# bcc-research/CFMMRouter.jl

Measured on AMD Instinct MI355X. Metric: find_arb! pools/sec + route! wall-clock, 1M-pool arbitrage, 1/2/4/8 GPU, higher is better.
Workload: dtype f64; 1 GPU; config3: 1M mixed ProductTwoCoin + GeometricMeanTwoCoin pools (500k each), 256 tokens, LinearNonnegative arbitrage; pools_per_gpu=1000000, pools_total=1000000, variant=materialising, full=False

## Files before the change

### cfmmrouter.jl_amd/csrc/ops_two_coin.h

```cpp
#pragma once

#include "fast_arith.h"

#include <type_traits>

namespace cfmm {

struct Trade {
    double d1, d2, l1, l2;
};

struct Px {
    double v1, v2, y1, y2, yg, dlv;
};

constexpr int kDirNone = 0, kDir1 = 1, kDir2 = 2, kDirBoth = 3;
__device__ __forceinline__ void expand_dir(int dir, double d, double l, Trade& t)
{
    if (dir == kDirBoth) return;
    t.d1 = dir == kDir1 ? d : 0.0;
    t.d2 = dir == kDir2 ? d : 0.0;
    t.l1 = dir == kDir2 ? l : 0.0;
    t.l2 = dir == kDir1 ? l : 0.0;
}

typedef unsigned int stream_u2 __attribute__((ext_vector_type(2), may_alias));
typedef unsigned int stream_u4 __attribute__((ext_vector_type(4), may_alias));
template <bool LEAN, class T, class I>
__device__ __forceinline__ T stream_at(const T* base, I i)
{
    if constexpr (LEAN) {
        static_assert(sizeof(T) == 8 || sizeof(T) == 16, "pool streams are 8- or 16-byte records");
        using Bits = typename std::conditional<sizeof(T) == 8, stream_u2, stream_u4>::type;
        const Bits bits = *reinterpret_cast<const Bits*>(reinterpret_cast<const char*>(base) + (size_t)((uint32_t)i * (uint32_t)sizeof(T)));
        T out;
        __builtin_memcpy(&out, &bits, sizeof(T));
        return out;
    } else {
        return base[i];
    }
}

template <bool LEAN = false, class I>
__device__ __forceinline__ int2 load_packed(const PackedFeeTok* pk, I i)
{
    const PackedFeeTok k = stream_at<LEAN>(pk, i);
    return make_int2((int)k.tok, (int)k.gidx);
}
__device__ __forceinline__ double load_packed_fee(int gbase, const double* fee) { return gbase < 0 ? *fee : 0.0; }
template <bool FAST, bool LEAN = false>
__device__ __forceinline__ void resolve_packed(int gbase, const double2* gtab_lds, int2& ai, double& g, double& yg)
{
    const unsigned tok = (unsigned)ai.x;
    if (LEAN || gbase >= 0) {
        const double2 gy = gtab_lds[gbase + ai.y];
        g = gy.x;
        yg = pinned(gy.y);
    } else if constexpr (FAST) {
        yg = rcp_refined(g);
    }
    ai = make_int2((int)(tok & 0xffffu), (int)(tok >> 16));
}

struct ProductOps {
    static constexpr bool kNeedsLogPrices = false;
    static constexpr bool kPrefetch = true;
    struct Raw {
        double2 R;
        double g;
        int2 ai;
        double yg;
    };
    ProductPools p;
    template <bool GBINS, bool LEAN = false, class I>
    __device__ __forceinline__ Raw load(I i) const
    {
        Raw r;
        r.R = stream_at<LEAN>(p.R, i);
        r.yg = 0.0;
        if constexpr (GBINS) {
            r.g = p.gamma[i];
            r.ai = p.Ai[i];
        } else {
            r.ai = load_packed<LEAN>(p.pk, i);
            r.g = LEAN ? 0.0 : load_packed_fee(p.gbase, p.gamma + i);
        }
        return r;
    }
    template <bool GBINS, bool FAST, bool LEAN = false>
    __device__ __forceinline__ void resolve(Raw& r, const double2* gtab_lds) const
    {
        if constexpr (!GBINS) resolve_packed<FAST, LEAN>(p.gbase, gtab_lds, r.ai, r.g, r.yg);
    }
    __device__ __forceinline__ int2 tokens(const Raw& r) const { return r.ai; }
    __device__ __forceinline__ void solve_full(double R1, double R2, double g, double v1, double v2, Trade& t) const
    {
        const double k = R1 * R2;
        const double m12 = v2 / v1;
        const double m21 = v1 / v2;
        const double gm12 = g * m12;
        const double gm21 = g * m21;
        t.d1 = max0(sqrt(gm12 * k) - R1) / g;
        t.d2 = max0(sqrt(gm21 * k) - R2) / g;
        t.l1 = max0(R1 - sqrt(k / gm21));
        t.l2 = max0(R2 - sqrt(k / gm12));
    }

    template <bool FAST>
    __device__ __forceinline__ int solve_dir(const Raw& r, const Px& px, double& d, double& l, Trade& t) const
    {
        const double R1 = r.R.x, R2 = r.R.y, g = r.g, v1 = px.v1, v2 = px.v2;
        constexpr double kMargin = 1.0 + 1e-12;
        const double a = v1 * R1, b = v2 * R2;
        const bool p1 = (g * b) * kMargin >= a;
        const bool p2 = (g * a) * kMargin >= b;
        d = l = 0.0;
        if (p1 != p2) {
            const double k = R1 * R2;
            const double r_in = p1 ? R1 : R2, r_out = p1 ? R2 : R1;
            if constexpr (FAST) {
                const double gm = g * div_by(p1 ? v2 : v1, p1 ? v1 : v2, p1 ? px.y1 : px.y2);
                d = div_by(__builtin_fmax(fast_sqrt(gm * k) - r_in, 0.0), g, px.yg);
                l = __builtin_fmax(r_out - fast_sqrt(fast_div(k, gm)), 0.0);
            } else {
                const double gm = g * ((p1 ? v2 : v1) / (p1 ? v1 : v2));
                d = max0(sqrt(gm * k) - r_in) / g;
                l = max0(r_out - sqrt(k / gm));
            }
            return p1 ? kDir1 : kDir2;
        }
        if (p1 || a != a || b != b) {
            solve_full(R1, R2, g, v1, v2, t);
            return kDirBoth;
        }
        return kDirNone;
    }
};

__device__ __forceinline__ double geom_arb_delta(double m, double r1, double r2, double eta, double g)
{
    const double inner = (((g * m) * eta) * r1) * pow(r2, eta);
    return max0(pow(inner, 1.0 / (eta + 1.0)) - r2) / g;
}
__device__ __forceinline__ double geom_arb_lambda(double m, double r1, double r2, double eta, double g)
{
    const double base = (r2 * pow(r1, 1.0 / eta)) / ((eta * g) * m);
    return max0(r1 - pow(base, eta / (1.0 + eta)));
}

struct GeoMeanOps {
    static constexpr bool kNeedsLogPrices = false;
    static constexpr bool kPrefetch = true;
    struct Raw {
        double2 R, w;
        double g;
        int2 ai;
        double yg;
    };
    GeoMeanPools p;
    template <bool GBINS, bool LEAN = false, class I>
    __device__ __forceinline__ Raw load(I i) const { return Raw{p.R[i], p.w[i], p.gamma[i], p.Ai[i], 0.0}; }
    template <bool GBINS, bool FAST, bool LEAN = false>
    __device__ __forceinline__ void resolve(Raw&, const double2*) const {}
    __device__ __forceinline__ int2 tokens(const Raw& r) const { return r.ai; }
    template <bool FAST>
    __device__ __forceinline__ int solve_dir(const Raw& r, const Px& px, double& d, double& l, Trade& t) const
    {
        d = l = 0.0;
        const double v1 = px.v1, v2 = px.v2;
        const double R1 = r.R.x, R2 = r.R.y, g = r.g;
        const double eta = r.w.x / r.w.y;
        const double ieta = 1.0 / eta;
        const double m12 = v2 / v1, m21 = v1 / v2;
        constexpr double kMargin = 1.0 + 1e-11;
        const bool p1 = (((g * m12) * eta) * R2) * kMargin >= R1;
        const bool p2 = (((g * m21) * ieta) * R1) * kMargin >= R2;
        t.d1 = t.d2 = t.l1 = t.l2 = 0.0;
        if (p1 != p2) {
            const double m = p1 ? m12 : m21, e = p1 ? eta : ieta;
            const double ra = p1 ? R2 : R1, rb = p1 ? R1 : R2;
            const double dx = geom_arb_delta(m, ra, rb, e, g);
            const double lx = geom_arb_lambda(m, ra, rb, e, g);
            t.d1 = p1 ? dx : 0.0;
            t.d2 = p1 ? 0.0 : dx;
            t.l1 = p1 ? 0.0 : lx;
            t.l2 = p1 ? lx : 0.0;
        } else if (p1) {
            t.d1 = geom_arb_delta(m12, R2, R1, eta, g);
            t.d2 = geom_arb_delta(m21, R1, R2, ieta, g);
            t.l1 = geom_arb_lambda(m21, R1, R2, ieta, g);
            t.l2 = geom_arb_lambda(m12, R2, R1, eta, g);
        }
        return kDirBoth;
    }
};

struct GeoMeanLogOps {
    static constexpr bool kNeedsLogPrices = true;
    static constexpr bool kPrefetch = true;
    struct Raw {
        double2 R, Q;
        double eta, g;
        int2 ai;
        double yg;
    };
    GeoMeanPools p;
    template <bool GBINS, bool LEAN = false, class I>
    __device__ __forceinline__ Raw load(I i) const
    {
        Raw r;
        r.R = stream_at<LEAN>(p.R, i);
        r.Q = stream_at<LEAN>(p.Q, i);
        r.eta = stream_at<LEAN>(p.eta, i);
        r.yg = 0.0;
        if constexpr (GBINS) {
            r.g = p.gamma[i];
            r.ai = p.Ai[i];
        } else {
            r.ai = load_packed<LEAN>(p.pk, i);
            r.g = LEAN ? 0.0 : load_packed_fee(p.gbase, p.gamma + i);
        }
        return r;
    }
    template <bool GBINS, bool FAST, bool LEAN = false>
    __device__ __forceinline__ void resolve(Raw& r, const double2* gtab_lds) const
    {
        if constexpr (!GBINS) resolve_packed<FAST, LEAN>(p.gbase, gtab_lds, r.ai, r.g, r.yg);
    }
    __device__ __forceinline__ int2 tokens(const Raw& r) const { return r.ai; }
    template <bool FAST>
    __device__ __forceinline__ void one_direction(const Raw& r, const Px& px, bool dir1, double n, double dd, double& d, double& l) const
    {
        const double R1 = r.R.x, R2 = r.R.y, g = r.g, eta = r.eta;
        const double ra = dir1 ? R2 : R1, rb = dir1 ? R1 : R2;
        const double A = dir1 ? (r.Q.x + px.dlv) : (r.Q.y - eta * px.dlv);
        double X, Y;
        if constexpr (FAST) {
            X = fast_exp(fast_div(A, eta + 1.0));
            Y = fast_div((X * ra) * dd, n);
            d = div_by(max0(X - rb), g, px.yg);
        } else {
            X = exp(A / (eta + 1.0));
            Y = ((X * ra) * dd) / n;
            d = max0(X - rb) / g;
        }
        l = max0(ra - Y);
    }
    template <bool FAST>
    __device__ __forceinline__ int solve_dir(const Raw& r, const Px& px, double& d, double& l, Trade& t) const
    {
        const double v1 = px.v1, v2 = px.v2;
        const double R1 = r.R.x, R2 = r.R.y, g = r.g;
        const double eta = r.eta;
        const double n1 = ((g * v2) * eta) * R2, d1 = v1;
        const double n2 = (g * v1) * R1, d2 = v2 * eta;
        const bool p1 = n1 > R1 * d1, p2 = n2 > R2 * d2;
        d = l = 0.0;
        if (v1 != v1 || v2 != v2) { t.d1 = t.d2 = t.l1 = t.l2 = v1 + v2; return kDirBoth; }
        if (!(p1 || p2)) return kDirNone;
        one_direction<FAST>(r, px, p1, p1 ? n1 : n2, p1 ? d1 : d2, d, l);
        if (!(p1 && p2)) return p1 ? kDir1 : kDir2;
        t.d1 = d;
        t.l2 = l;
        one_direction<FAST>(r, px, false, n2, d2, t.d2, t.l1);
        return kDirBoth;
    }
};

struct SolidlyOps : ProductOps {
    template <bool FAST>
    __device__ __forceinline__ int solve_dir(const Raw& r, const Px& px, double& d, double& l, Trade& t) const
    {
        const double R1 = r.R.x, R2 = r.R.y, g = r.g, v1 = px.v1, v2 = px.v2;
        d = l = 0.0;
        if (v1 != v1 || v2 != v2) { t.d1 = t.d2 = t.l1 = t.l2 = v1 + v2; return kDirBoth; }
        const double s1 = R1 * R1, s2 = R2 * R2;
        const double A = v2 * (R2 * __builtin_fma(3.0, s1, s2));
        const double B = v1 * (R1 * __builtin_fma(3.0, s2, s1));
        const bool p1 = g * A > B, p2 = A < g * B;
        if (!(p1 || p2)) return kDirNone;
        const double va = p1 ? v1 : v2, vb = p1 ? v2 : v1;
        const double ra = p1 ? R1 : R2, rb = p1 ? R2 : R1;
        const double num = __builtin_fma(-g, vb, va), den = __builtin_fma(g, vb, va);
        const double c = cbrt(num / den);
        const double c2 = c * c;
        const double tt = (va * ((1.0 + c) + c2)) / ((g * vb) * ((1.0 - c) + c2));
        const double t0 = rb / ra;
        const double rho = (t0 * __builtin_fma(t0, t0, 1.0)) / (tt * __builtin_fma(tt, tt, 1.0));
        const double xa = ra * sqrt(sqrt(rho));
        d = max0(xa - ra) / g;
        l = max0(rb - tt * xa);
        return p1 ? kDir1 : kDir2;
    }
};

}
```

### cfmmrouter.jl_amd/csrc/sweep_core.h

```cpp
#pragma once

#include "granule.h"
#include "ops_two_coin.h"
#include "ops_univ3.h"

#include <type_traits>

namespace cfmm {

typedef double d2v __attribute__((ext_vector_type(2)));
__device__ __forceinline__ void store_pair(double2* dst, double x, double y, int nt)
{
    d2v val = {x, y};
    if (nt) asm volatile("global_store_dwordx4 %0, %1, off nt\n\ts_nop 1" : : "v"(dst), "v"(val) : "memory");
    else asm volatile("global_store_dwordx4 %0, %1, off sc1\n\ts_nop 1" : : "v"(dst), "v"(val) : "memory");
}
__device__ __forceinline__ void store_pair_at(double2* base, uint32_t i, double x, double y)
{
    d2v val = {x, y};
    asm volatile("s_nop 4\n\tglobal_store_dwordx4 %0, %1, %2 sc1\n\ts_nop 1" : : "v"(i * 16u), "v"(val), "s"(base) : "memory");
}

__device__ __forceinline__ void store_row(double* dst, double x)
{
    asm volatile("global_store_dwordx2 %0, %1, off sc1" : : "v"(dst), "v"(x) : "memory");
}

struct SweepLds {
    double2* vy;
    double2* gtab;
    double* lv;
    double* bins;
    double* wsum;
    double* flags;
    double* my_bins;
};

template <int BLOCK, bool GBINS>
__device__ __forceinline__ SweepLds carve_lds(const SweepArgs& a)
{
    extern __shared__ __attribute__((aligned(16))) double lds[];
    SweepLds L;
    if constexpr (GBINS) {
        L.vy = nullptr;
        L.gtab = nullptr;
        L.lv = L.bins = L.my_bins = L.flags = nullptr;
        L.wsum = lds;
        return L;
    }
    L.vy = reinterpret_cast<double2*>(lds);
    L.gtab = reinterpret_cast<double2*>(lds + ((size_t)a.n_pad << (a.v_shift - 3)));
    L.lv = reinterpret_cast<double*>(L.gtab + a.gtab_n);
    L.bins = L.lv + (a.need_logv ? a.n_pad : 0);
    L.wsum = L.bins + (size_t)a.copies * a.n_pad;
    L.flags = L.wsum + BLOCK / 64;
    L.my_bins = L.bins + (size_t)(a.copies == 1 ? 0 : (threadIdx.x >> 6)) * a.n_pad;
    return L;
}

__device__ __forceinline__ int wait_armed(const SweepArgs& a)
{
    const long long t0 = (long long)wall_clock64();
    for (;;) {
        const unsigned long long w = __hip_atomic_load(a.arm_word, __ATOMIC_RELAXED, __HIP_MEMORY_SCOPE_SYSTEM);
        if (w == a.arm_seq) return 1;
        if ((w & ~kArmCancel) > a.arm_seq || w == (a.arm_seq | kArmCancel)) return 0;
        if ((long long)wall_clock64() - t0 > a.arm_timeout) return -1;
        __builtin_amdgcn_s_sleep(1);
    }
}

__device__ __forceinline__ void report(const SweepArgs& a, unsigned long long bit)
{
    if (a.flags && threadIdx.x == 0) __hip_atomic_fetch_or(a.flags, bit, __ATOMIC_RELAXED, __HIP_MEMORY_SCOPE_SYSTEM);
}

constexpr int kStageLive = 1, kStageFast = 2, kStageGaveUp = 4;
constexpr int kPricePre = 2;
struct PricePre {
    double p[kPricePre];
};
template <int BLOCK>
__device__ __forceinline__ PricePre request_prices(const double* v, int n)
{
    PricePre r;
#pragma unroll
    for (int k = 0; k < kPricePre; ++k) {
        const int j = (int)threadIdx.x + k * BLOCK;
        r.p[k] = v[j < n ? j : n - 1];
    }
    return r;
}
template <int BLOCK, bool GBINS, bool PRE = false>
__device__ __forceinline__ int stage_prices(const SweepArgs& a, const SweepLds& L, const PricePre& pre = PricePre{})
{
    if constexpr (GBINS) {
        __syncthreads();
        return kStageLive;
    }
    const int tid = threadIdx.x;
    const int n_zero = a.copies * a.n_pad;
    const bool logs = a.need_logv != 0;
    const bool armed = a.arm_word != nullptr;
    bool live = true, gave_up = false;
    if (armed) {
        for (int j = tid; j < n_zero; j += BLOCK) L.bins[j] = 0.0;
        for (int j = tid; j < a.gtab_n; j += BLOCK) {
            const double g = a.gtab[j];
            L.gtab[j] = make_double2(g, rcp_refined(g));
        }
        if (tid == 0) L.flags[BLOCK / 64] = (double)wait_armed(a);
        __syncthreads();
        live = L.flags[BLOCK / 64] > 0.0;
        gave_up = L.flags[BLOCK / 64] < 0.0;
    }
    bool in_window = true;
    for (int j = tid, k = 0; j < a.n; j += BLOCK, ++k) {
        double vj;
        if (armed) vj = __hip_atomic_load(a.v + j, __ATOMIC_RELAXED, __HIP_MEMORY_SCOPE_SYSTEM);
        else if (PRE && k < kPricePre) vj = k == 0 ? pre.p[0] : pre.p[1];
        else vj = a.v[j];
        if (a.v_shift == 4) L.vy[j] = make_double2(vj, rcp_refined(vj));
        else reinterpret_cast<double*>(L.vy)[j] = vj;
        in_window = in_window && in_fast_window(vj);
        if (logs) L.lv[j] = log(vj);
    }
    if (!armed) {
        for (int j = tid; j < n_zero; j += BLOCK) L.bins[j] = 0.0;
        for (int j = tid; j < a.gtab_n; j += BLOCK) {
            const double g = a.gtab[j];
            L.gtab[j] = make_double2(g, rcp_refined(g));
        }
    }
    const bool wave_in = __all(in_window ? 1 : 0) != 0;
    if ((tid & 63) == 0) L.flags[tid >> 6] = wave_in ? 1.0 : 0.0;
    __syncthreads();
    bool all_in = true;
#pragma unroll
    for (int w = 0; w < BLOCK / 64; ++w) all_in = all_in && L.flags[w] != 0.0;
    return (live ? kStageLive : 0) | (all_in ? kStageFast : 0) | (gave_up ? kStageGaveUp : 0);
}

template <class Ops, bool MAT, bool GBINS, bool FAST, bool LEAN, class Idx>
__device__ __forceinline__ void process_pool(const Ops& ops, const SweepArgs& a, const SweepLds& L,
                                             const typename Ops::Raw& raw_in, Idx i, double& acc)
{
    const auto put_record = [&](double x, double y) {
        if constexpr (LEAN) store_pair_at(a.Delta, i, x, y);
        else store_pair(a.Delta + i, x, y, a.nt_stores);
    };
    typename Ops::Raw raw = raw_in;
    ops.template resolve<GBINS, FAST, LEAN>(raw, L.gtab);
    const int2 tok = ops.tokens(raw);
    Px px;
    px.yg = raw.yg;
    if constexpr (GBINS) {
        px.v1 = a.v[tok.x];
        px.v2 = a.v[tok.y];
        px.y1 = px.y2 = 0.0;
        px.dlv = Ops::kNeedsLogPrices ? log(px.v2 / px.v1) : 0.0;
    } else {
        if constexpr (FAST) {
            const double2 a1 = L.vy[tok.x], a2 = L.vy[tok.y];
            px.v1 = a1.x; px.y1 = a1.y;
            px.v2 = a2.x; px.y2 = a2.y;
        } else {
            const char* base = reinterpret_cast<const char*>(L.vy);
            px.v1 = *reinterpret_cast<const double*>(base + ((size_t)tok.x << a.v_shift));
            px.v2 = *reinterpret_cast<const double*>(base + ((size_t)tok.y << a.v_shift));
            px.y1 = px.y2 = 0.0;
        }
        px.dlv = 0.0;
        if constexpr (Ops::kNeedsLogPrices)
            px.dlv = a.need_logv ? L.lv[tok.y] - L.lv[tok.x] : log(px.v2 / px.v1);
    }
    Trade t;
    double d, l;
    int dir;
    dir = ops.template solve_dir<FAST>(raw, px, d, l, t);
    const double v1 = px.v1, v2 = px.v2;
    const bool one = dir == kDir1 || dir == kDir2;
    const bool plain = one && (!MAT || !a.compact || (__double2hiint(d) | __double2hiint(l)) >= 0);
    if (plain) {
        const bool d1 = dir == kDir1;
        if (MAT) {
            if (a.compact) {
                put_record(d1 ? d : -d, l);
            } else {
                store_pair(a.Delta + i, d1 ? d : 0.0, d1 ? 0.0 : d, a.nt_stores);
                store_pair(a.Lambda + i, d1 ? 0.0 : l, d1 ? l : 0.0, a.nt_stores);
            }
        }
        acc += l * (d1 ? v2 : v1) - d * (d1 ? v1 : v2);
        if constexpr (GBINS) {
            a.gflow[i] = d1 ? make_double2(0.0 - d, l) : make_double2(l, 0.0 - d);
        } else {
            const double f_in = 0.0 - d;
            if (f_in != 0.0) atomicAdd(&L.my_bins[d1 ? tok.x : tok.y], f_in);
            if (l != 0.0) atomicAdd(&L.my_bins[d1 ? tok.y : tok.x], l);
        }
        return;
    }
    if (dir == kDirNone) {
        if (MAT) {
            if (a.compact) {
                put_record(0.0, 0.0);
            } else {
                store_pair(a.Delta + i, 0.0, 0.0, a.nt_stores);
                store_pair(a.Lambda + i, 0.0, 0.0, a.nt_stores);
            }
        }
        if constexpr (GBINS) a.gflow[i] = make_double2(0.0, 0.0);
        return;
    }
    expand_dir(dir, d, l, t);
    if (MAT) {
        if (a.compact) {
            const int d1h = __double2hiint(t.d1), d2h = __double2hiint(t.d2), l1h = __double2hiint(t.l1), l2h = __double2hiint(t.l2);
            const int z1 = d2h | __double2loint(t.d2) | l1h | __double2loint(t.l1);
            const int z2 = d1h | __double2loint(t.d1) | l2h | __double2loint(t.l2);
            const bool dir1 = (z1 == 0) & ((d1h | l2h) >= 0);
            const bool dir2 = (z2 == 0) & ((d2h | l1h) >= 0);
            double ra = t.d1, rb = t.l2;
            if (!dir1) {
                if (dir2) {
                    ra = -t.d2;
                    rb = t.l1;
                } else {
                    a.Lambda[i] = make_double2(t.d1, t.d2);
                    a.Over[i] = make_double2(t.l1, t.l2);
                    ra = 0.0;
                    rb = -1.0;
                }
            }
            put_record(ra, rb);
        } else {
            store_pair(a.Delta + i, t.d1, t.d2, a.nt_stores);
            store_pair(a.Lambda + i, t.l1, t.l2, a.nt_stores);
        }
    }
    acc += (t.l1 * v1 + t.l2 * v2) - (t.d1 * v1 + t.d2 * v2);
    const double f1 = t.l1 - t.d1, f2 = t.l2 - t.d2;
    if constexpr (GBINS) {
        a.gflow[i] = make_double2(f1, f2);
    } else {
        if (f1 != 0.0) atomicAdd(&L.my_bins[tok.x], f1);
        if (f2 != 0.0) atomicAdd(&L.my_bins[tok.y], f2);
    }
}

template <class Ops, bool MAT, int BLOCK, bool GBINS, bool FAST, bool PREFETCH, bool LEAN, class Idx>
__device__ __forceinline__ void tile_loop(const Ops& ops, const SweepArgs& a, const SweepLds& L, typename Ops::Raw cur,
                                          Idx i, Idx step, Idx left, double& acc)
{
    if constexpr (PREFETCH) {
        bool ok = left > 0;
        while (ok) {
            const bool more = left > 1;
            typename Ops::Raw nxt = cur;
            if (more) nxt = ops.template load<GBINS, LEAN>((Idx)(i + step));
            process_pool<Ops, MAT, GBINS, FAST, LEAN>(ops, a, L, cur, i, acc);
            i += step;
            --left;
            ok = more;
            cur = nxt;
        }
    } else {
        bool ok = left > 0;
        while (ok) {
            process_pool<Ops, MAT, GBINS, FAST, LEAN>(ops, a, L, cur, i, acc);
            i += step;
            ok = --left > 0;
            if (ok) cur = ops.template load<GBINS, LEAN>(i);
        }
    }
}

constexpr int kArithFull = 0, kArithFast = 1, kArithAuto = 2;
template <class Ops, bool MAT, int BLOCK, bool GBINS, int FASTK, bool MULTI, bool LEAN, class Idx>
__device__ __forceinline__ double sweep_tiles(const Ops& ops, const SweepArgs& a, const SweepLds& L, const typename Ops::Raw& cur,
                                              Idx i, Idx step, Idx left, bool& poison, bool& live, const PricePre& pre)
{
    static_assert(!(GBINS && FASTK != kArithFull), "large-market mode runs on the compiler's sequences");
    double acc = 0.0;
    const int staged = stage_prices<BLOCK, GBINS, !GBINS>(a, L, pre);
    poison = (staged & kStageLive) == 0;
    live = !poison || (staged & kStageGaveUp) != 0;
    if (staged & kStageGaveUp) report(a, kFlagGaveUp);
    if (FASTK == kArithFast && !poison && (staged & kStageFast) == 0) {
        poison = true;
        report(a, kFlagWindow);
    }
    if (poison) left = 0;
    constexpr bool kPre = Ops::kPrefetch && !MULTI;
    if constexpr (FASTK == kArithAuto) {
        if (staged & kStageFast) tile_loop<Ops, MAT, BLOCK, GBINS, true, kPre, LEAN>(ops, a, L, cur, i, step, left, acc);
        else tile_loop<Ops, MAT, BLOCK, GBINS, false, kPre, LEAN>(ops, a, L, cur, i, step, left, acc);
    } else {
        tile_loop<Ops, MAT, BLOCK, GBINS, FASTK == kArithFast, kPre, LEAN>(ops, a, L, cur, i, step, left, acc);
    }
    return acc;
}

typedef unsigned long long u2v __attribute__((ext_vector_type(2)));
__device__ __forceinline__ void publish_column(const SweepArgs& a, int j, double val)
{
    if (a.direct_host.gran) {
        u2v g = {granule(a.direct_host.tag, val, 0), granule(a.direct_host.tag, val, 1)};
        asm volatile("global_store_dwordx4 %0, %1, off sc0 sc1\n\ts_nop 1" : : "v"(a.direct_host.gran + 2 * (size_t)j), "v"(g) : "memory");
    } else {
        a.direct_out[j] = val;
    }
}

template <int BLOCK, bool GBINS>
__device__ __forceinline__ void finish_row(const SweepArgs& a, const SweepLds& L, double acc, int row_id, bool poison, bool publish)
{
    const double nan = __builtin_nan("");
    if (poison) acc = nan;
    constexpr int kWaves = BLOCK / 64;
    const int tid = threadIdx.x;
    const int wave = tid >> 6;
#pragma unroll
    for (int off = 32; off > 0; off >>= 1) acc += __shfl_down(acc, off, 64);
    if ((tid & 63) == 0) L.wsum[wave] = acc;
    __syncthreads();

    const int n_cols = GBINS ? 0 : a.n;
    if (!GBINS && a.direct) {
        if (!publish) return;
        for (int j = tid; j < n_cols; j += BLOCK) {
            double s = L.bins[j];
            for (int c = 1; c < a.copies; ++c) s += L.bins[(size_t)c * a.n_pad + j];
            publish_column(a, j, poison ? nan : s);
        }
        if (tid == 0) {
            double s = L.wsum[0];
            for (int w = 1; w < kWaves; ++w) s += L.wsum[w];
            publish_column(a, n_cols, poison ? nan : s);
        }
        return;
    }
    double* row = a.partials + (size_t)row_id * a.row_pitch;
    for (int j = tid; j < n_cols; j += BLOCK) {
        double s = L.bins[j];
        for (int c = 1; c < a.copies; ++c) s += L.bins[(size_t)c * a.n_pad + j];
        store_row(row + j, poison ? nan : s);
    }
    if (tid == 0) {
        double s = L.wsum[0];
        for (int w = 1; w < kWaves; ++w) s += L.wsum[w];
        store_row(row + n_cols, poison ? nan : s);
    }
}

#define CFMM_CONST_AS __attribute__((address_space(4)))
template <class T>
__device__ __forceinline__ const CFMM_CONST_AS T* const_as(const T* p)
{
    return (const CFMM_CONST_AS T*)(reinterpret_cast<uintptr_t>(p));
}
struct LaunchHead {
    const SweepDesc* desc;
    const double* v;
    int reverse;
    int n;
};
static_assert(offsetof(SweepLaunch, desc) == 0 && offsetof(SweepLaunch, v) == 8 && offsetof(SweepLaunch, reverse) == 16 &&
                  offsetof(SweepLaunch, n) == 20 && offsetof(SweepLaunch, tail) == 24 && alignof(SweepTail) == 8,
              "sweep_kernel / sweep_multi (pointer, pointer, int, int, SweepTail) read the segment as a SweepLaunch");
typedef const CFMM_CONST_AS SweepLaunch& LaunchRef;
__device__ __forceinline__ LaunchRef launch_args()
{
    return *(const CFMM_CONST_AS SweepLaunch*)__builtin_amdgcn_kernarg_segment_ptr();
}
__device__ __forceinline__ BlockRec block_rec(const SweepDesc* desc)
{
    const CFMM_CONST_AS BlockRec* recs =
        (const CFMM_CONST_AS BlockRec*)(reinterpret_cast<uintptr_t>(desc) + kSweepDescHead);
    const CFMM_CONST_AS BlockRec& r = recs[blockIdx.x];
    return BlockRec{r.first, r.stride, r.full, r.tail, r.row, r.seg, r.kind};
}
__device__ __forceinline__ SweepArgs block_args(const LaunchHead& h, LaunchRef la, const CFMM_CONST_AS SweepDesc& d,
                                                const CFMM_CONST_AS SegRec& sg)
{
    const CFMM_CONST_AS SweepTail& t = la.tail;
    SweepArgs a;
    a.v = la.v;
    a.n = d.n;
    a.n_pad = d.n_pad;
    a.v_shift = d.v_shift;
    a.need_logv = d.need_logv;
    a.gtab = d.gtab;
    a.gtab_n = d.gtab_n;
    a.copies = d.copies;
    a.flags = d.flags;
    a.m = sg.m;
    a.Delta = sg.Delta;
    a.Lambda = sg.Lambda;
    a.Over = sg.Over;
    a.compact = d.compact;
    a.partials = d.partials;
    a.row_pitch = d.row_pitch;
    a.gflow = sg.gflow;
    a.reverse = h.reverse;
    a.arm_word = t.arm_word;
    a.arm_seq = t.arm_seq;
    a.arm_timeout = t.arm_timeout;
    a.nt_stores = d.nt_stores;
    a.direct = d.direct;
    a.direct_out = t.direct_out;
    a.direct_host = HostOut{t.direct_host.gran, t.direct_host.tag};
    return a;
}
__device__ __forceinline__ ProductPools pools_of(const CFMM_CONST_AS AnyPools& u, const ProductPools*)
{
    return ProductPools{u.p.R, u.p.gamma, u.p.Ai, u.p.pk, u.p.gbase};
}
__device__ __forceinline__ GeoMeanPools pools_of(const CFMM_CONST_AS AnyPools& u, const GeoMeanPools*)
{
    return GeoMeanPools{u.g.R, u.g.w, u.g.gamma, u.g.Ai, u.g.eta, u.g.Q, u.g.reference_order, u.g.pk, u.g.gbase};
}
__device__ __forceinline__ UniV3Pools pools_of(const CFMM_CONST_AS AnyPools& u, const UniV3Pools*)
{
    return UniV3Pools{u.u.pg, u.u.Ai, u.u.cur_a, u.u.cur_b, u.u.cur_c, u.u.curR, u.u.walk, u.u.ticks, u.u.thr, u.u.head,
                      u.u.has_walk, u.u.cp, u.u.pk, u.u.gbase};
}
template <class Ops, bool MAT, int BLOCK, bool GBINS, int FASTK, bool MULTI, bool LEAN>
__device__ __forceinline__ void sweep_body(const LaunchHead& h, const CFMM_CONST_AS SweepDesc& d, const CFMM_CONST_AS SegRec& sg,
                                           const BlockRec& br, const PricePre& pre)
{
    static_assert(!(LEAN && (GBINS || FASTK == kArithFull)), "the lean kernels: LDS bins, prices staged as pairs");
    using Idx = typename std::conditional<LEAN, uint32_t, int64_t>::type;
    const Ops ops{pools_of(sg.pools, (const decltype(Ops::p)*)nullptr)};
    const int64_t stride = br.stride;
    const int64_t i0 = br.first + threadIdx.x;
    const int64_t left = br.full + ((int)threadIdx.x < br.tail ? 1 : 0);
    const bool reverse = h.reverse != 0;
    const int64_t step = reverse ? -stride : stride;
    const int64_t i = reverse ? i0 + (left - 1) * stride : i0;
    typename Ops::Raw cur = {};
    if (left > 0) cur = ops.template load<GBINS, LEAN>((Idx)i);
    SweepArgs a = block_args(h, launch_args(), d, sg);
    if constexpr (LEAN) {
        a.compact = 1;
        a.nt_stores = 0;
        a.v_shift = 4;
        a.copies = BLOCK / 64;
        a.direct = 0;
    }
    const SweepLds L = carve_lds<BLOCK, GBINS>(a);
    if constexpr (LEAN) a.need_logv = Ops::kNeedsLogPrices ? 1 : 0;
    bool poison, live;
    const double acc = sweep_tiles<Ops, MAT, BLOCK, GBINS, FASTK, MULTI, LEAN>(ops, a, L, cur, (Idx)i, (Idx)step, (Idx)left, poison, live, pre);
    finish_row<BLOCK, GBINS>(a, L, acc, br.row, poison, live);
}

template <class Ops, bool MAT, int BLOCK, bool GBINS, int FASTK, bool LEAN = false>
__global__ __launch_bounds__(BLOCK) void sweep_kernel(const SweepDesc* desc, const double* v, int reverse, int n, SweepTail)
{
    const LaunchHead h{desc, v, reverse, n};
    PricePre pre = {};
    if constexpr (!GBINS) pre = request_prices<BLOCK>(v, n);
    const BlockRec br = block_rec(desc);
    const CFMM_CONST_AS SweepDesc& d = *const_as(desc);
    sweep_body<Ops, MAT, BLOCK, GBINS, FASTK, false, LEAN>(h, d, d.seg[0], br, pre);
}

template <bool MAT, int BLOCK, bool GBINS, int FASTK, bool LEAN = false>
__global__ __launch_bounds__(BLOCK) void sweep_multi(const SweepDesc* desc, const double* v, int reverse, int n, SweepTail)
{
    const LaunchHead h{desc, v, reverse, n};
    PricePre pre = {};
    if constexpr (!GBINS) pre = request_prices<BLOCK>(v, n);
    const BlockRec br = block_rec(desc);
    const CFMM_CONST_AS SweepDesc& d = *const_as(desc);
    const CFMM_CONST_AS SegRec& sg = d.seg[br.seg];
    switch (br.kind) {
    case 0: sweep_body<ProductOps, MAT, BLOCK, GBINS, FASTK, true, LEAN>(h, d, sg, br, pre); break;
    case 1:
        sweep_body<GeoMeanLogOps, MAT, BLOCK, GBINS, FASTK, true, LEAN>(h, d, sg, br, pre);
        break;
    default: sweep_body<UniV3Ops, MAT, BLOCK, GBINS, FASTK, true, LEAN>(h, d, sg, br, pre); break;
    }
}
#undef CFMM_CONST_AS

}
```

Measured before the change: 79.35 billion pools/s.

## Add lean per-pool fast path for product and log-geomean pools with rare fallback

Adds a branch-light lean_solve for ProductOps and GeoMeanLogOps that computes a single-direction trade. It detects rare cases (both directions, NaN, negative outputs) with a wave-wide vote and sends only those to the full finish_pool path. The lean path decodes packed token indices and the gamma table inline, and compresses the flag check in stage_prices to paired reads. The aim is to cut branching, register pressure and generic record logic in the hot loop, at the cost of a margin-based direction test that could shift borderline pools into the slow path.

```diff
diff --git a/cfmmrouter.jl_amd/csrc/ops_two_coin.h b/cfmmrouter.jl_amd/csrc/ops_two_coin.h
--- a/cfmmrouter.jl_amd/csrc/ops_two_coin.h
+++ b/cfmmrouter.jl_amd/csrc/ops_two_coin.h
@@ -134,6 +134,33 @@
             return kDirBoth;
         }
         return kDirNone;
+    }
+    template <bool FAST>
+    __device__ __forceinline__ void lean_solve(const Raw& r, const Px& px, double& d, double& l, bool& dir1, bool& trades, bool& rare) const
+    {
+        const double R1 = r.R.x, R2 = r.R.y, g = r.g, v1 = px.v1, v2 = px.v2;
+        constexpr double kMargin = 1.0 + 1e-12;
+        const double a = v1 * R1, b = v2 * R2;
+        const bool p1 = (g * b) * kMargin >= a;
+        const bool p2 = (g * a) * kMargin >= b;
+        trades = p1 != p2;
+        dir1 = !p2;
+        rare = (p1 == p2) & (p1 | (a != a) | (b != b));
+        d = l = 0.0;
+        if (trades) {
+            const double k = R1 * R2;
+            const double r_in = p1 ? R1 : R2, r_out = p1 ? R2 : R1;
+            const double v_in = p1 ? v1 : v2, v_out = p1 ? v2 : v1;
+            if constexpr (FAST) {
+                const double gm = g * div_by(v_out, v_in, p1 ? px.y1 : px.y2);
+                d = div_by(__builtin_fmax(fast_sqrt(gm * k) - r_in, 0.0), g, px.yg);
+                l = __builtin_fmax(r_out - fast_sqrt(fast_div(k, gm)), 0.0);
+            } else {
+                const double gm = g * (v_out / v_in);
+                d = max0(sqrt(gm * k) - r_in) / g;
+                l = max0(r_out - sqrt(k / gm));
+            }
+        }
     }
 };
 
@@ -265,6 +292,36 @@
         one_direction<FAST>(r, px, false, n2, d2, t.d2, t.l1);
         return kDirBoth;
     }
+    template <bool FAST>
+    __device__ __forceinline__ void lean_solve(const Raw& r, const Px& px, double& d, double& l, bool& dir1, bool& trades, bool& rare) const
+    {
+        const double v1 = px.v1, v2 = px.v2;
+        const double R1 = r.R.x, R2 = r.R.y, g = r.g, eta = r.eta;
+        const double n1 = ((g * v2) * eta) * R2, d1 = v1;
+        const double n2 = (g * v1) * R1, d2 = v2 * eta;
+        const bool p1 = n1 > R1 * d1, p2 = n2 > R2 * d2;
+        trades = p1 | p2;
+        dir1 = !p2;
+        rare = (p1 & p2) | (v1 != v1) | (v2 != v2);
+        d = l = 0.0;
+        if (trades) {
+            const double A1 = r.Q.x + px.dlv, A2 = r.Q.y - eta * px.dlv;
+            const double A = p1 ? A1 : A2;
+            const double ra = p1 ? R2 : R1, rb = p1 ? R1 : R2;
+            const double n = p1 ? n1 : n2, dd = p1 ? d1 : d2;
+            double X, Y;
+            if constexpr (FAST) {
+                X = fast_exp(fast_div(A, eta + 1.0));
+                Y = fast_div((X * ra) * dd, n);
+                d = div_by(max0(X - rb), g, px.yg);
+            } else {
+                X = exp(A / (eta + 1.0));
+                Y = ((X * ra) * dd) / n;
+                d = max0(X - rb) / g;
+            }
+            l = max0(ra - Y);
+        }
+    }
 };
 
 struct SolidlyOps : ProductOps {
diff --git a/cfmmrouter.jl_amd/csrc/sweep_core.h b/cfmmrouter.jl_amd/csrc/sweep_core.h
--- a/cfmmrouter.jl_amd/csrc/sweep_core.h
+++ b/cfmmrouter.jl_amd/csrc/sweep_core.h
@@ -91,7 +91,7 @@
     }
     return r;
 }
-template <int BLOCK, bool GBINS, bool PRE = false>
+template <int BLOCK, bool GBINS, bool PRE = false, bool LEAN = false>
 __device__ __forceinline__ int stage_prices(const SweepArgs& a, const SweepLds& L, const PricePre& pre = PricePre{})
 {
     if constexpr (GBINS) {
@@ -136,44 +136,31 @@
     if ((tid & 63) == 0) L.flags[tid >> 6] = wave_in ? 1.0 : 0.0;
     __syncthreads();
     bool all_in = true;
+    if constexpr (LEAN) {
+        static_assert((BLOCK / 64) % 2 == 0, "flags are read in pairs");
+        const double2* pairs = reinterpret_cast<const double2*>(L.flags);
+        int bits = -1;
 #pragma unroll
-    for (int w = 0; w < BLOCK / 64; ++w) all_in = all_in && L.flags[w] != 0.0;
+        for (int w = 0; w < BLOCK / 128; ++w) {
+            const double2 f = pairs[w];
+            bits &= __double2hiint(f.x) & __double2hiint(f.y);
+        }
+        all_in = bits != 0;
+    } else {
+#pragma unroll
+        for (int w = 0; w < BLOCK / 64; ++w) all_in = all_in && L.flags[w] != 0.0;
+    }
     return (live ? kStageLive : 0) | (all_in ? kStageFast : 0) | (gave_up ? kStageGaveUp : 0);
 }
 
 template <class Ops, bool MAT, bool GBINS, bool FAST, bool LEAN, class Idx>
-__device__ __forceinline__ void process_pool(const Ops& ops, const SweepArgs& a, const SweepLds& L,
-                                             const typename Ops::Raw& raw_in, Idx i, double& acc)
+__device__ __forceinline__ void finish_pool(const Ops& ops, const SweepArgs& a, const SweepLds& L, const typename Ops::Raw& raw,
+                                            const Px& px, int2 tok, Idx i, double& acc)
 {
     const auto put_record = [&](double x, double y) {
         if constexpr (LEAN) store_pair_at(a.Delta, i, x, y);
         else store_pair(a.Delta + i, x, y, a.nt_stores);
     };
-    typename Ops::Raw raw = raw_in;
-    ops.template resolve<GBINS, FAST, LEAN>(raw, L.gtab);
-    const int2 tok = ops.tokens(raw);
-    Px px;
-    px.yg = raw.yg;
-    if constexpr (GBINS) {
-        px.v1 = a.v[tok.x];
-        px.v2 = a.v[tok.y];
-        px.y1 = px.y2 = 0.0;
-        px.dlv = Ops::kNeedsLogPrices ? log(px.v2 / px.v1) : 0.0;
-    } else {
-        if constexpr (FAST) {
-            const double2 a1 = L.vy[tok.x], a2 = L.vy[tok.y];
-            px.v1 = a1.x; px.y1 = a1.y;
-            px.v2 = a2.x; px.y2 = a2.y;
-        } else {
-            const char* base = reinterpret_cast<const char*>(L.vy);
-            px.v1 = *reinterpret_cast<const double*>(base + ((size_t)tok.x << a.v_shift));
-            px.v2 = *reinterpret_cast<const double*>(base + ((size_t)tok.y << a.v_shift));
-            px.y1 = px.y2 = 0.0;
-        }
-        px.dlv = 0.0;
-        if constexpr (Ops::kNeedsLogPrices)
-            px.dlv = a.need_logv ? L.lv[tok.y] - L.lv[tok.x] : log(px.v2 / px.v1);
-    }
     Trade t;
     double d, l;
     int dir;
@@ -249,6 +236,83 @@
     }
 }
 
+template <class Ops> struct HasLeanSolve : std::false_type {};
+template <> struct HasLeanSolve<ProductOps> : std::true_type {};
+template <> struct HasLeanSolve<GeoMeanLogOps> : std::true_type {};
+
+template <class Ops, bool MAT, bool FAST, class Idx>
+__device__ __forceinline__ void process_pool_lean(const Ops& ops, const SweepArgs& a, const SweepLds& L,
+                                                  const typename Ops::Raw& raw_in, Idx i, double& acc)
+{
+    typename Ops::Raw raw = raw_in;
+    const unsigned packed = (unsigned)raw.ai.x;
+    const int2 tok = make_int2((int)(packed & 0xffffu), (int)(packed >> 16));
+    const double2 gy = L.gtab[ops.p.gbase + raw.ai.y];
+    const double2 a1 = L.vy[tok.x], a2 = L.vy[tok.y];
+    double g = gy.x, yg = gy.y, v1 = a1.x, y1 = a1.y, v2 = a2.x, y2 = a2.y, lv1 = 0.0, lv2 = 0.0;
+    if constexpr (Ops::kNeedsLogPrices) {
+        lv1 = L.lv[tok.x];
+        lv2 = L.lv[tok.y];
+        asm volatile("" : "+v"(g), "+v"(yg), "+v"(v1), "+v"(y1), "+v"(v2), "+v"(y2), "+v"(lv1), "+v"(lv2));
+    } else {
+        asm volatile("" : "+v"(g), "+v"(yg), "+v"(v1), "+v"(y1), "+v"(v2), "+v"(y2));
+    }
+    raw.ai = tok;
+    raw.g = g;
+    raw.yg = yg;
+    const Px px{v1, v2, y1, y2, yg, lv2 - lv1};
+    double d, l;
+    bool dir1, trades, rare;
+    ops.template lean_solve<FAST>(raw, px, d, l, dir1, trades, rare);
+    if (MAT) rare = rare | ((__double2hiint(d) | __double2hiint(l)) < 0);
+    if (__builtin_expect(__any(rare ? 1 : 0) != 0, 0)) {
+        finish_pool<Ops, MAT, false, FAST, true>(ops, a, L, raw, px, tok, i, acc);
+        return;
+    }
+    if (MAT) store_pair_at(a.Delta, i, dir1 ? d : -d, l);
+    const double worth = l * (dir1 ? v2 : v1) - d * (dir1 ? v1 : v2);
+    acc = trades ? acc + worth : acc;
+    const double f_in = 0.0 - d;
+    if (f_in != 0.0) atomicAdd(&L.my_bins[dir1 ? tok.x : tok.y], f_in);
+    if (l != 0.0) atomicAdd(&L.my_bins[dir1 ? tok.y : tok.x], l);
+}
+
+template <class Ops, bool MAT, bool GBINS, bool FAST, bool LEAN, class Idx>
+__device__ __forceinline__ void process_pool(const Ops& ops, const SweepArgs& a, const SweepLds& L,
+                                             const typename Ops::Raw& raw_in, Idx i, double& acc)
+{
+    if constexpr (LEAN && HasLeanSolve<Ops>::value) {
+        process_pool_lean<Ops, MAT, FAST>(ops, a, L, raw_in, i, acc);
+        return;
+    }
+    typename Ops::Raw raw = raw_in;
+    ops.template resolve<GBINS, FAST, LEAN>(raw, L.gtab);
+    const int2 tok = ops.tokens(raw);
+    Px px;
+    px.yg = raw.yg;
+    if constexpr (GBINS) {
+        px.v1 = a.v[tok.x];
+        px.v2 = a.v[tok.y];
+        px.y1 = px.y2 = 0.0;
+        px.dlv = Ops::kNeedsLogPrices ? log(px.v2 / px.v1) : 0.0;
+    } else {
+        if constexpr (FAST) {
+            const double2 a1 = L.vy[tok.x], a2 = L.vy[tok.y];
+            px.v1 = a1.x; px.y1 = a1.y;
+            px.v2 = a2.x; px.y2 = a2.y;
+        } else {
+            const char* base = reinterpret_cast<const char*>(L.vy);
+            px.v1 = *reinterpret_cast<const double*>(base + ((size_t)tok.x << a.v_shift));
+            px.v2 = *reinterpret_cast<const double*>(base + ((size_t)tok.y << a.v_shift));
+            px.y1 = px.y2 = 0.0;
+        }
+        px.dlv = 0.0;
+        if constexpr (Ops::kNeedsLogPrices)
+            px.dlv = a.need_logv ? L.lv[tok.y] - L.lv[tok.x] : log(px.v2 / px.v1);
+    }
+    finish_pool<Ops, MAT, GBINS, FAST, LEAN>(ops, a, L, raw, px, tok, i, acc);
+}
+
 template <class Ops, bool MAT, int BLOCK, bool GBINS, bool FAST, bool PREFETCH, bool LEAN, class Idx>
 __device__ __forceinline__ void tile_loop(const Ops& ops, const SweepArgs& a, const SweepLds& L, typename Ops::Raw cur,
                                           Idx i, Idx step, Idx left, double& acc)
@@ -283,7 +347,7 @@
 {
     static_assert(!(GBINS && FASTK != kArithFull), "large-market mode runs on the compiler's sequences");
     double acc = 0.0;
-    const int staged = stage_prices<BLOCK, GBINS, !GBINS>(a, L, pre);
+    const int staged = stage_prices<BLOCK, GBINS, !GBINS, LEAN>(a, L, pre);
     poison = (staged & kStageLive) == 0;
     live = !poison || (staged & kStageGaveUp) != 0;
     if (staged & kStageGaveUp) report(a, kFlagGaveUp);
```

Measured after the change: 82.98 billion pools/s, median of 6. +4.6%, better.
